# pypr/pysph

Hardware: AMD Instinct MI355X
Metric: particle-updates/sec (nnps.update + AccelerationEval.compute), WCSPH 3D, fp64 (higher is better)
Workload: dtype f64

## Files before the change

pysph_amd/csrc/sph_eval.hip:

```cpp
#include "sph_internal.h"
#include "sph_kernels.h"
#include "sph_pair.h"

#include <cfloat>
#include <cmath>
#include <type_traits>

struct EosArgs {
    int kind;
    double par[SPH_MAX_PAR];
    double *rho, *p, *cs;
    size_t start, stop;
    double *q[SPH_PROP_COUNT];
    uint32_t *tflag;
};

__device__ inline void jacobi_eigen3(double A[3][3], double V[3][3], double d[3])
{
    for (int i = 0; i < 3; i++) for (int j = 0; j < 3; j++) V[i][j] = (i == j) ? 1.0 : 0.0;
    for (int sweep = 0; sweep < 12; sweep++) {
        double off = fabs(A[0][1]) + fabs(A[0][2]) + fabs(A[1][2]);
        double diag = fabs(A[0][0]) + fabs(A[1][1]) + fabs(A[2][2]);
        if (off <= 1e-300 || off <= 1e-18 * diag) break;
#pragma unroll
// ... 334 lines not shown
    }
    const double rho = v[6];
    const double q = rho != 0.0 ? v[7] * (1.0 / (rho * rho)) : 0.0;
    const double srho = ((a.cls >> sl) & 1u) ? -rho : rho;
    if (!(rho > 0.0) && fabs(v[0]) < SPH_PARKED_MIN) atomicOr(a.rho_flag, 1u);
    double hp = 0.0;
    if (VH) hp = kernarg_read<const double *>(__builtin_offsetof(PackMArgs, prop) + ((size_t)8 * SPH_MAX_ARRAYS + sl) * sizeof(double *))[o];
    a.fpos[i] = make_float4((float)(v[0] - a.gmin[0]), (float)(v[1] - a.gmin[1]), (float)(v[2] - a.gmin[2]),
                            VH ? (float)(a.hr * hp) : (float)a.hr);
    double2 pc[PACK_MAXP];
#pragma unroll
    for (int k = 0; k < PACK_MAXP; k++) pc[k] = make_double2(0.0, 0.0);
    int np;
    if (VH && F32) {
        pc[0] = __builtin_bit_cast(double2, make_float4((float)(v[0] - a.gmin[0]), (float)(v[1] - a.gmin[1]), (float)(v[2] - a.gmin[2]), (float)hp));
        pc[1] = __builtin_bit_cast(double2, make_float4((float)v[3], (float)v[4], (float)v[5], (float)srho));
        np = 2;
    } else if (VH) {
        pc[0] = make_double2(v[0], v[1]); pc[1] = make_double2(v[2], hp);
        pc[2] = make_double2(v[3], v[4]); pc[3] = make_double2(v[5], srho);
        np = 4;
    } else if (F32) {
        pc[0] = __builtin_bit_cast(double2, make_float4((float)(v[0] - a.gmin[0]), (float)(v[1] - a.gmin[1]), (float)(v[2] - a.gmin[2]), (float)v[3]));
        pc[1] = __builtin_bit_cast(double2, make_float4((float)v[4], (float)v[5], (float)srho, (float)q));
        np = 2;
    } else {
        pc[0] = make_double2(v[0], v[1]); pc[1] = make_double2(v[2], v[3]);
        pc[2] = make_double2(v[4], v[5]); pc[3] = make_double2(srho, q);
        np = 4;
    }
    emit_pieces(a, i, pc, np);
}

template <class T> struct FamWCSPH_T {
    typedef T Real;
    static constexpr uint32_t CF0 = F_CONT | F_MOM | F_XSPH;
#ifndef SPH_WCSPH_MINB
#define SPH_WCSPH_MINB 4
#endif
    static constexpr int MINB = SPH_WCSPH_MINB;
    static constexpr int NA = 8;
    static constexpr int NR = 12;
    struct Params {
        T c0, alpha, beta, gx, gy, gz, eps;
        double *arho, *au, *av, *aw, *ax, *ay, *az, *dt_cfl, *dt_force;
    };
    struct Dest {
        T u, v, w, rho, p, cs, tmpi;
        T arho, au, av, aw, ax, ay, az, dt_cfl;
    };
    template <class A> static __device__ __forceinline__ void load(Dest &D, const T *a, const A &, uint32_t)
    {
        D.u = a[0]; D.v = a[1]; D.w = a[2]; D.rho = a[4]; D.tmpi = a[5]; D.cs = a[6]; D.p = a[7];
        D.arho = D.au = D.av = D.aw = D.ax = D.ay = D.az = T(0.0);
        D.dt_cfl = T(-1.0);
    }
    static constexpr bool PRED = true;
    template <int KK, bool UH, class A>
    static __device__ __forceinline__ void pair(Dest &D, const real4<T> &pi, const real4<T> &pj, T r2,
                                                const T (&s)[NA], uint32_t fl, const A &a, bool pass = true)
    {
        PairGeomT<T> g;
        constexpr bool MRG = SPH_MERGED_RSQ && sizeof(T) == 8 && KK != 4;
        T tt_m = T(0.0);
        if constexpr (MRG) {
            if (fl & F_MOM) tt_m = pair_geom_mom<KK, UH>(g, pi, pj, r2, T(0.5) * (D.rho + s[4]), a);
            else pair_geom<KK, UH>(g, pi, pj, r2, a);
        } else {
            pair_geom<KK, UH>(g, pi, pj, r2, a);
        }
        const T tg = pair_gradfac<KK, UH>(g);
        const T vij0 = D.u - s[0], vij1 = D.v - s[1], vij2 = D.w - s[2];
        const T vdotx = vij0 * g.xij[0] + vij1 * g.xij[1] + vij2 * g.xij[2];
        const T mj = pass ? s[3] : T(0.0);
        if (fl & F_CONT) D.arho = fma(mj * tg, vdotx, D.arho);
        if (fl & (F_MOM | F_XSPH)) {
            const T rhoij = T(0.5) * (D.rho + s[4]);
            T rhoij1;
            T wij = T(0.0);
            if (fl & (F_XSPH | F_TENSILE)) wij = pair_w<KK, UH>(g);
            if (fl & F_MOM) {
                const T re = r2 + g.eps;
                const T tt = MRG ? tt_m : fast_rcp(re * rhoij);
                const T inv_re = rhoij * tt;
                rhoij1 = re * tt;
                const T hv = g.hij * vdotx;
                const T muij = raw_min(hv, T(0.0)) * inv_re;
                const T cij = T(0.5) * (D.cs + s[6]);
                const T piij = (a.p.beta * muij - a.p.alpha * cij) * muij * rhoij1;
                const T dtv = fabs(hv * (g.rinv * g.rinv));
                D.dt_cfl = raw_max(D.dt_cfl, (r2 > T(1e-12) && pass) ? dtv : T(-1.0));
                const T tmpj = s[5];
                T tmp = D.tmpi + tmpj;
                if (fl & F_TENSILE) {
                    const T qd = (a.k.deltap * g.hij) * g.h1;
                    const T wdp = SphKernel<KK>::w(qd) * g.fac;
                    T fij = wij * fast_rcp(wdp);
                    fij = fij * fij;
                    fij = fij * fij;
                    const T Ri = D.p > 0 ? T(0.01) * D.tmpi : T(0.2) * fabs(D.tmpi);
                    const T Rj = s[7] > 0 ? T(0.01) * tmpj : T(0.2) * fabs(tmpj);
                    tmp = (D.tmpi + tmpj) + (Ri + Rj) * fij;
                }
                const T ft = -mj * (tmp + piij) * tg;
                D.au = fma(ft, g.xij[0], D.au);
                D.av = fma(ft, g.xij[1], D.av);
                D.aw = fma(ft, g.xij[2], D.aw);
            } else {
                rhoij1 = fast_rcp(rhoij);
            }
            if (fl & F_XSPH) {
                const T tmp = -a.p.eps * mj * wij * rhoij1;
                D.ax = fma(tmp, vij0, D.ax);
                D.ay = fma(tmp, vij1, D.ay);
                D.az = fma(tmp, vij2, D.az);
            }
        }
    }
    template <class A> static __device__ __forceinline__ void finish(Dest &D, const A &a, uint32_t o)
    {
        if (a.dflags & F_CONT) a.p.arho[o] = D.arho;
        if (a.dflags & F_MOM) {
            T au = D.au + a.p.gx, av = D.av + a.p.gy, aw = D.aw + a.p.gz;
            a.p.au[o] = au; a.p.av[o] = av; a.p.aw[o] = aw;
            a.p.dt_cfl[o] = D.dt_cfl < T(0.0) ? T(0.0) : D.dt_cfl + a.p.c0;
            a.p.dt_force[o] = au * au + av * av + aw * aw;
        }
        if (a.dflags & F_XSPH) {
            a.p.ax[o] = D.ax + D.u; a.p.ay[o] = D.ay + D.v; a.p.az[o] = D.az + D.w;
        }
    }
};
typedef FamWCSPH_T<double> FamWCSPH;

template <class T, bool UM = false> struct FamWCSPHE_T : FamWCSPH_T<T> {
    static constexpr bool EOSF = true;
    static constexpr bool UMASS = UM;
    static constexpr int NR = 8;
    struct Raw {
        typename std::conditional<sizeof(T) == 8, double2, float4>::type q[sizeof(T) == 8 ? 4 : 2];
    };
    template <class A> static __device__ __forceinline__ void load_raw(const A &a, uint32_t jg, Raw &r)
    {
        if constexpr (sizeof(T) == 8) {
            const double2 *p = reinterpret_cast<const double2 *>(a.rec) + (unsigned long long)jg * 4;
            r.q[0] = p[0]; r.q[1] = p[1]; r.q[2] = p[2]; r.q[3] = p[3];
        } else {
            const float4 *p = reinterpret_cast<const float4 *>(a.rec) + (unsigned long long)jg * 2;
            r.q[0] = p[0]; r.q[1] = p[1];
        }
    }
    template <class A> static __device__ __forceinline__ void decode(const A &a, const Raw &r, uint32_t fl, T mu, real4<T> &pj, T (&s)[8],
                                                                     int gk = 3)
    {
        T rho;
        if constexpr (sizeof(T) == 8) {
            pj.x = r.q[0].x; pj.y = r.q[0].y; pj.z = r.q[1].x; pj.w = 0.0;
            s[0] = r.q[1].y; s[1] = r.q[2].x; s[2] = r.q[2].y; s[3] = r.q[3].y; rho = r.q[3].x;
        } else {
            pj.x = r.q[0].x; pj.y = r.q[0].y; pj.z = r.q[0].z; pj.w = 0.f;
            s[0] = r.q[0].w; s[1] = r.q[1].x; s[2] = r.q[1].y; s[3] = r.q[1].w; rho = r.q[1].z;
        }
        s[4] = rho;
        s[5] = s[6] = s[7] = T(0.0);
        if constexpr (UM) {
            const T q = s[3];
            s[3] = mu;
            if (fl & F_MOM) {
                const T ratio = rho * (T)a.e_rho01;
                s[5] = q;
                s[6] = (T)a.e_c0 * tait_cs_power(ratio, gk);
            }
        } else
        if (fl & F_MOM) {
            const T ratio = rho * (T)a.e_rho01;
            T r7, r3;
            tait_powers(ratio, gk, r7, r3);
            const T p = (T)a.e_p0 + (T)a.e_B * (r7 - T(1.0));
            s[5] = rho != T(0.0) ? p * fast_rcp(rho * rho) : T(0.0);
            s[6] = (T)a.e_c0 * r3;
            s[7] = p;
        }
    }
    template <class A> static __device__ __forceinline__ void load_fused(const A &a, uint32_t jg, uint32_t fl, T mu, real4<T> &pj, T (&s)[8])
    {
        Raw r;
        load_raw(a, jg, r);
        decode(a, r, fl, mu, pj, s);
    }
};

template <class T, bool UM = false> struct FamWCSPHEG_T : FamWCSPHE_T<T, UM> {
    typedef FamWCSPHE_T<T, UM> Base;
    template <class A> static __device__ __forceinline__ void load_fused(const A &a, uint32_t jg, uint32_t fl, T mu, real4<T> &pj, T (&s)[8])
    {
        typename Base::Raw r;
        Base::load_raw(a, jg, r);
        Base::decode(a, r, fl, mu, pj, s, a.e_gk);
    }
};

template <class T> struct FamWCSPHV_T : FamWCSPH_T<T> {
    static constexpr bool EOSF = true;
    static constexpr int NR = 8;
    template <class A> static __device__ __forceinline__ void load_fused(const A &a, uint32_t jg, uint32_t fl, T mu, real4<T> &pj, T (&s)[8])
    {
        T rho;
        if constexpr (sizeof(T) == 8) {
            const double2 *p = reinterpret_cast<const double2 *>(a.rec) + (unsigned long long)jg * 4;
            const double2 q0 = p[0], q1 = p[1], q2 = p[2], q3 = p[3];
            pj.x = q0.x; pj.y = q0.y; pj.z = q1.x; pj.w = q1.y;
            s[0] = q2.x; s[1] = q2.y; s[2] = q3.x; rho = q3.y;
        } else {
            const float4 *p = reinterpret_cast<const float4 *>(a.rec) + (unsigned long long)jg * 2;
            const float4 q0 = p[0], q1 = p[1];
            pj.x = q0.x; pj.y = q0.y; pj.z = q0.z; pj.w = q0.w;
            s[0] = q1.x; s[1] = q1.y; s[2] = q1.z; rho = q1.w;
        }
        s[3] = mu;
        s[4] = rho;
// ... 550 lines not shown
    uint32_t o = a.d_perm[i];
    if (o < a.d_start || o >= a.d_stop) return;
    double4 pi = a.posh[a.d_off + i];
    typename Fam::Dest D;
    Fam::load(D, a.aux + (size_t)(a.d_off + i) * Fam::NA, a, o);
    uint32_t key = a.d_keys[i];
    int cx = key % a.nc[0];
    int t = key / a.nc[0];
    int cy = t % a.nc[1], cz = t / a.nc[1];
    double hi2 = a.radius_scale * pi.w;
    hi2 *= hi2;
    for (int s = 0; s < a.nsrc; s++) {
        const SrcDesc sd = a.src[s];
        for (int oz = -1; oz <= 1; oz++)
            for (int oy = -1; oy <= 1; oy++) {
                int yy = cy + oy, zz = cz + oz;
                if (yy < 0 || yy >= a.nc[1] || zz < 0 || zz >= a.nc[2]) continue;
                int xa = max(cx - 1, 0), xb = min(cx + 1, a.nc[0] - 1);
                uint32_t row = (uint32_t)(a.nc[0] * (yy + a.nc[1] * zz));
                uint32_t j0 = sd.cell_start[row + xa], j1 = sd.cell_start[row + xb + 1];
                for (uint32_t j = j0; j < j1; j++) {
                    double4 pj = a.posh[sd.off + j];
                    double hj2 = a.radius_scale * pj.w;
                    hj2 *= hj2;
                    double r2 = r2_exact(pi.x - pj.x, pi.y - pj.y, pi.z - pj.z);
                    if ((r2 < hi2) || (r2 < hj2)) {
                        double sj[Fam::NA];
                        load_aux<Fam>(sj, a.aux + (size_t)(sd.off + j) * Fam::NA);
                        Fam::template pair<KK, UH>(D, pi, pj, r2, sj, sd.flags, a);
                    }
                }
            }
    }
    Fam::finish(D, a, o);
}

static bool is_nosrc_kind(int k)
{
    return k == SPH_EQ_TAIT_EOS || k == SPH_EQ_TAIT_EOS_HG || k == SPH_EQ_TVF_STATE_EQUATION ||
           k == SPH_EQ_ISOTHERMAL_EOS || k == SPH_EQ_SOLID_ISOTHERMAL_EOS || k == SPH_EQ_MONAGHAN_ART_STRESS ||
           k == SPH_EQ_HOOKES_DEVIATORIC_STRESS_RATE;
}

static int need_prop(sph_ctx *c, int id, int prop, const char *who)
{
    if (!c->arr[id].prop[prop]) {
        sph_set_error("%s: array %d has no device copy of a required property (id %d); push it first", who, id, prop);
        return SPH_ERR_MISSING_PROP;
    }
    return SPH_OK;
}

static int run_nosrc(sph_ctx *c, const sph_equation &e, size_t start, size_t stop)
{
    if (stop <= start) return SPH_OK;
    DevArray &A = c->arr[e.dest];
    EosArgs a;
    a.kind = e.kind;
    memcpy(a.par, e.par, sizeof a.par);
    SPH_TRY(need_prop(c, e.dest, SPH_RHO, "EOS"));
    SPH_TRY(sph_array_ensure_prop(c, e.dest, SPH_P));
    a.rho = A.prop[SPH_RHO];
    a.p = A.prop[SPH_P];
    a.cs = nullptr;
    if (e.kind == SPH_EQ_TAIT_EOS || e.kind == SPH_EQ_TAIT_EOS_HG) {
        SPH_TRY(sph_array_ensure_prop(c, e.dest, SPH_CS));
        a.cs = A.prop[SPH_CS];
// ... 267 lines not shown
        case 3: LAUNCH(3); break;
        case 4: LAUNCH(4); break;
        }
#undef LAUNCH
        return SPH_OK;
    }
}

template <class Fam, bool UHV = true> static int launch_pair_fused(sph_ctx *c, int kk, const PairArgs<Fam> &a)
{
    if (a.nd == 0) return SPH_OK;
    constexpr bool FP32 = sizeof(typename Fam::Real) == 4;
    dim3 g2(div_up(4 * div_up(a.nd, 256), WPB)), b2(64 * WPB);
    uint32_t cf = a.src[0].flags;
    for (int j = 1; j < a.nsrc; j++) if (a.src[j].flags != cf) cf = 0;
    if (c->const_flags == 0) cf = 0;
    if constexpr (fam_rowlds<Fam>::value && UHV) {
        if (c->row_lds && !a.nl_mode && !a.face_mode) {
            dim3 g1(4 * div_up(a.nd, 256)), b1(64);
#define LAUNCHL(K)                                                                                              \
            if (cf == Fam::CF0) hipLaunchKernelGGL((k_pair_rowlds<Fam, K, Fam::CF0>), g1, b1, 0, c->stream, a); \
            else hipLaunchKernelGGL((k_pair_rowlds<Fam, K, 0>), g1, b1, 0, c->stream, a)
            switch (kk) {
            case 1: LAUNCHL(1); break;
            case 2: LAUNCHL(2); break;
            case 3: LAUNCHL(3); break;
            case 4: LAUNCHL(4); break;
            }
#undef LAUNCHL
            c->timers[T_N_ROWLDS].count++;
            return SPH_OK;
        }
    }
#define LAUNCHE(K)                                                                                                              \
    if (cf == Fam::CF0) hipLaunchKernelGGL((k_pair_wave<Fam, K, UHV, FP32, Fam::CF0>), g2, b2, (size_t)c->lds_pad, c->stream, a); \
    else hipLaunchKernelGGL((k_pair_wave<Fam, K, UHV, FP32, 0>), g2, b2, (size_t)c->lds_pad, c->stream, a)
    switch (kk) {
    case 1: LAUNCHE(1); break;
    case 2: LAUNCHE(2); break;
    case 3: LAUNCHE(3); break;
    case 4: LAUNCHE(4); break;
    }
#undef LAUNCHE
    return SPH_OK;
}

template <class Fam>
static void fill_common(sph_ctx *c, PairArgs<Fam> &a, const sph_kernel *K, double t)
{
    a.posh = c->posh.as<double4>();
    a.aux = c->aux.as<double>();
    a.rec = c->posh.as<double>();
    a.nrec = c->cur_nrec;
    a.fpos = c->fposb.as<float4>();
    a.dom_extent = fmax(fmax(c->xmax[0] - c->xmin[0], c->xmax[1] - c->xmin[1]), c->xmax[2] - c->xmin[2]);
    for (int k = 0; k < 3; k++) { a.nc[k] = c->nc[k]; a.xmin[k] = c->xmin[k]; }
    a.cell_size = c->cell_size;
    a.radius_scale = c->radius_scale;
    a.k.sigma = K->fac;
    a.k.deltap = K->deltap;
    a.k.dim = K->dim;
    a.t = t;
    a.dt = c->cur_dt;
    a.ablate = (int)c->ablate;
    a.dbg = c->count_iters ? c->dbgc.as<unsigned long long>() : nullptr;
    a.hu = 0.5 * (c->h_uniform + c->h_uniform);
    a.h1u = 1.0 / a.hu;
    a.facu = K->fac * a.h1u;
// ... 485 lines not shown
                const DevArray &S = c->arr[srcs[j]];
                a.src[a.nsrc++] = {S.cell_start.as<uint32_t>(), (uint32_t)off_of[j], sflags[j], S.fine_start.as<uint32_t>(), S.m_value, 0u};
            }
            for (int j = 0; j < nsrcs && phase != 1; j++) {
                const DevArray &S = c->arr[srcs[j]];
                if (S.g_n == 0) continue;
                a.src[a.nsrc++] = {S.g_cell_start.as<uint32_t>(), (uint32_t)(off_of[j] + S.n_binned), sflags[j],
                                   S.g_fine_start.as<uint32_t>(), S.m_value, 1u};
            }
            a.face_mode = c->split_pair ? phase : 0;
            a.d_off = (uint32_t)d_off; a.nd = (uint32_t)D.n_binned;
            a.d_mu = D.m_value;
            a.d_keys = D.keys_sorted.as<uint32_t>(); a.d_fkeys = D.fkeys_sorted.as<uint32_t>(); a.d_perm = D.perm.as<uint32_t>();
            set_tile_order(c, a, D);
            a.d_start = (uint32_t)start; a.d_stop = (uint32_t)stop; a.dflags = dflags;
            a.nl = nullptr; a.nl_mode = nl_mode;
            if (nl_mode) a.nl = c->nlbuf.as<uint32_t>();
            if (start == 0 && stop == D.n_real && D.n_binned == D.n && !any_ghosts) use_dest_list(c, a, D);
            if (eosf || eosv) {
                a.e_rho01 = 1.0 / g->eos_par[0]; a.e_c0 = g->eos_par[1];
                a.e_B = g->eos_par[0] * g->eos_par[1] * g->eos_par[1] / g->eos_par[2];
        a.e_gk = tait_gk(g->eos_par[2]);
                a.e_p0 = g->eos_par[3];
            }
            if (tvff) { a.e_p0 = g->eos_par[0]; a.e_rho01 = 1.0 / g->eos_par[1]; a.e_B = g->eos_par[2]; }
        };
        auto run_wcsph = [&](auto tag) -> int {
            typedef decltype(tag) F;
            PairArgs<F> a;
            memset(&a, 0, sizeof a);
            common(a);
            const sph_equation *me = eq_of[SPH_EQ_MOMENTUM], *xe = eq_of[SPH_EQ_XSPH];
            if (me) { a.p.c0 = me->par[0]; a.p.alpha = me->par[1]; a.p.beta = me->par[2]; a.p.gx = me->par[3]; a.p.gy = me->par[4]; a.p.gz = me->par[5]; }
            if (xe) a.p.eps = xe->par[0];
            if (dflags & F_CONT) { SPH_TRY(ensure_out(c, dst, {SPH_ARHO})); a.p.arho = D.prop[SPH_ARHO]; }
            if (dflags & F_MOM) {
                SPH_TRY(ensure_out(c, dst, {SPH_AU, SPH_AV, SPH_AW, SPH_DT_CFL, SPH_DT_FORCE}));
                a.p.au = D.prop[SPH_AU]; a.p.av = D.prop[SPH_AV]; a.p.aw = D.prop[SPH_AW];
                a.p.dt_cfl = D.prop[SPH_DT_CFL]; a.p.dt_force = D.prop[SPH_DT_FORCE];
            }
            if (dflags & F_XSPH) {
                SPH_TRY(ensure_out(c, dst, {SPH_AX, SPH_AY, SPH_AZ}));
                a.p.ax = D.prop[SPH_AX]; a.p.ay = D.prop[SPH_AY]; a.p.az = D.prop[SPH_AZ];
            }
            if constexpr (std::is_same<F, FamWCSPHV_T<typename F::Real>>::value) return launch_pair_fused<F, false>(c, K->kind, a);
            else if constexpr (fam_eosf<F>::value) return launch_pair_fused<F>(c, K->kind, a);
            else return launch_pair<F>(c, K->kind, a);
        };
        auto run_density = [&](auto tag) -> int {
            typedef decltype(tag) F;
            PairArgs<F> a;
            memset(&a, 0, sizeof a);
            common(a);
            SPH_TRY(ensure_out(c, dst, {SPH_RHO}));
            a.p.rho = D.prop[SPH_RHO];
            if (dflags & F_TVFSD) { SPH_TRY(ensure_out(c, dst, {SPH_VOL})); a.p.V = D.prop[SPH_VOL]; }
            if ((dflags & F_SD) && (dflags & F_TVFSD)) { sph_set_error("both SummationDensity flavours on one destination"); return SPH_ERR_UNSUPPORTED; }
            return launch_pair<F>(c, K->kind, a);
        };
        auto run_vgrad = [&](auto tag) -> int {
            typedef decltype(tag) F;
            PairArgs<F> a;
            memset(&a, 0, sizeof a);
            common(a);
            static const int vp[9] = {SPH_V00, SPH_V01, SPH_V02, SPH_V10, SPH_V11, SPH_V12, SPH_V20, SPH_V21, SPH_V22};
            if ((dflags & F_VG2) && (dflags & F_VG3)) { sph_set_error("both VelocityGradient2D and 3D on one destination"); return SPH_ERR_UNSUPPORTED; }
// ... 356 lines not shown
```

pysph_amd/csrc/sph_kernels.h:

```cpp
#pragma once

#include <hip/hip_runtime.h>

template <int KIND> struct SphKernel;

__device__ __forceinline__ double raw_max(double a, double b)
{
    double r;
    asm("v_max_f64 %0, %1, %2" : "=v"(r) : "v"(a), "v"(b));
    return r;
}
__device__ __forceinline__ double raw_min(double a, double b)
{
    double r;
    asm("v_min_f64 %0, %1, %2" : "=v"(r) : "v"(a), "v"(b));
    return r;
}
__device__ __forceinline__ float raw_max(float a, float b) { return fmaxf(a, b); }
__device__ __forceinline__ float raw_min(float a, float b) { return fminf(a, b); }


template <class R> __device__ __forceinline__ R kernel_norm(R sigma, R h1, int dim)
{
    R f = sigma * h1;
    if (dim > 1) f *= h1;
    if (dim > 2) f *= h1;
    return f;
}

template <> struct SphKernel<1> {
    static constexpr bool HAS_DWQ = false;
    template <bool INSUP = false, class R> static __device__ __forceinline__ R dwq(R) { return R(0); }
    template <bool INSUP = false, class R> static __device__ __forceinline__ R w(R q)
    {
        R t2 = R(2) - q;
        R a = R(0.25) * t2 * t2 * t2;
        R b = R(1) - R(1.5) * q * q * (R(1) - R(0.5) * q);
        return (!INSUP && q > R(2)) ? R(0) : (q > R(1) ? a : b);
    }
    template <bool INSUP = false, class R> static __device__ __forceinline__ R dw(R q)
    {
        R t2 = R(2) - q;
        R a = R(-0.75) * t2 * t2;
        R b = R(-3) * q * (R(1) - R(0.75) * q);
        return (!INSUP && q > R(2)) ? R(0) : (q > R(1) ? a : b);
    }
};

template <> struct SphKernel<2> {
    static constexpr bool HAS_DWQ = true;
    template <bool INSUP = false, class R> static __device__ __forceinline__ R dwq(R q)
    {
// ... 48 lines not shown
```

pysph_amd/csrc/sph_pair.h:

```cpp
#pragma once

#include <hip/hip_runtime.h>
#include <cstdint>

#include "sphhip.h"
#include "sph_kernels.h"

template <class T> __device__ __forceinline__ T r2_exact(T dx, T dy, T dz)
{
#pragma clang fp contract(off)
    const T a = dx * dx, b = dy * dy, c = dz * dz;
    return (a + b) + c;
}

template <class T> struct Real4Of;
template <> struct Real4Of<double> { typedef double4 type; };
template <> struct Real4Of<float> { typedef float4 type; };
template <class T> using real4 = typename Real4Of<T>::type;


struct KernelConst {
    double sigma;
    double deltap;
    int dim;
// ... 33 lines not shown
    SrcDesc src[SPH_MAX_ARRAYS];
    const double4 *posh;
    const double *aux;
    const double *rec;
    int nrec;
    const float4 *fpos;
    double dom_extent;
    uint32_t d_off, nd;
    double d_mu;
    const uint32_t *d_keys, *d_fkeys, *d_perm;
    const uint8_t *d_slot;
    const uint32_t *d_tile_order;
    const uint32_t *d_list;
    int face_mode, gfx_lo, gfx_hi;
    int row_mod3;
    uint32_t d_start, d_stop;
    int nc[3];
    double xmin[3];
    double cell_size;
    double radius_scale;
    KernelConst k;
    uint32_t dflags;
    unsigned long long *dbg;
    int ablate;
    int skip_init;
    int skip_post;
    double t, dt;
    double hu, h1u, facu, epsu, hr2u;
    uint32_t *nl;
    int nl_mode;
    int norm_masks;
    double e_rho01, e_c0, e_B, e_p0;
    int e_gk;
    typename Fam::Params p;
};

template <class F, class = void> struct fam_merged { static constexpr bool value = false; };
template <class F> struct fam_merged<F, decltype((void)F::MERGED)> { static constexpr bool value = F::MERGED; };

template <class V> __device__ __forceinline__ V kernarg_read(size_t byte_offset)
{
    typedef const char __attribute__((address_space(4))) *kptr;
    const kptr ka = (kptr)__builtin_amdgcn_kernarg_segment_ptr();
    return *reinterpret_cast<const V __attribute__((address_space(4))) *>(ka + byte_offset);
}

template <class F, class = void> struct fam_token { static constexpr bool value = false; };
template <class F> struct fam_token<F, decltype((void)F::TOKEN)> { static constexpr bool value = F::TOKEN; };

template <class F, class = void> struct fam_eosf { static constexpr bool value = false; };
template <class F> struct fam_eosf<F, decltype((void)F::EOSF)> { static constexpr bool value = F::EOSF; };


#ifndef SPH_NEWTON_STEPS
#define SPH_NEWTON_STEPS 1
#endif
__device__ __forceinline__ double fast_rcp(double d)
{
    double x = __builtin_amdgcn_rcp(d);
    double e = fma(-d, x, 1.0);
    x = fma(x, e, x);
    if (SPH_NEWTON_STEPS > 1) {
        e = fma(-d, x, 1.0);
        x = fma(x, e, x);
    }
    return x;
}
__device__ __forceinline__ void fast_sqrt_rsqrt(double a, double &s, double &rs)
{
    a = raw_max(a, 1e-300);
    double y = __builtin_amdgcn_rsq(a);
    double g = a * y, h = 0.5 * y;
    double r = fma(-h, g, 0.5);
    g = fma(g, r, g);
    h = fma(h, r, h);
    if (SPH_NEWTON_STEPS > 1) {
        r = fma(-h, g, 0.5);
        g = fma(g, r, g);
        h = fma(h, r, h);
    }
    s = g;
    rs = h + h;
}
__device__ __forceinline__ float fast_rcp(float d) { return __builtin_amdgcn_rcpf(d); }
__device__ __forceinline__ void fast_sqrt_rsqrt(float a, float &s, float &rs)
{
    a = fmaxf(a, 1e-35f);
    rs = __builtin_amdgcn_rsqf(a);
    s = a * rs;
}

template <class T> struct PairGeomT {
    T xij[3];
    T r2, rij, rinv, hij, h1, q, fac, eps;
};
typedef PairGeomT<double> PairGeom;

template <int KK, bool UH, class T, class A>
__device__ __forceinline__ void pair_geom(PairGeomT<T> &g, const real4<T> &pi, const real4<T> &pj, T r2, const A &a)
{
    g.xij[0] = pi.x - pj.x; g.xij[1] = pi.y - pj.y; g.xij[2] = pi.z - pj.z;
    g.r2 = r2;
    constexpr bool EXACT_Q = (KK == 4);
    if (EXACT_Q) {
        g.rij = sqrt(r2);
        g.rinv = g.rij > T(0) ? T(1) / g.rij : T(0);
    } else {
        fast_sqrt_rsqrt(r2, g.rij, g.rinv);
    }
    if (UH) {
        g.hij = (T)a.hu; g.h1 = (T)a.h1u; g.fac = (T)a.facu; g.eps = (T)a.epsu;
    } else {
        g.hij = T(0.5) * (pi.w + pj.w);
        g.h1 = EXACT_Q ? T(1) / g.hij : fast_rcp(g.hij);
        g.fac = kernel_norm((T)a.k.sigma, g.h1, a.k.dim);
        g.eps = T(0.01) * g.hij * g.hij;
    }
    g.q = g.rij * g.h1;
}
#ifndef SPH_MERGED_RSQ
#define SPH_MERGED_RSQ 0
#endif
template <int KK, bool UH, class A>
__device__ __forceinline__ double pair_geom_mom(PairGeomT<double> &g, const double4 &pi, const double4 &pj, double r2, double rhoij, const A &a)
{
    typedef double T;
    g.xij[0] = pi.x - pj.x; g.xij[1] = pi.y - pj.y; g.xij[2] = pi.z - pj.z;
    g.r2 = r2;
    if (UH) {
        g.hij = (T)a.hu; g.h1 = (T)a.h1u; g.fac = (T)a.facu; g.eps = (T)a.epsu;
    } else {
        g.hij = T(0.5) * (pi.w + pj.w);
        g.h1 = fast_rcp(g.hij);
        g.fac = kernel_norm((T)a.k.sigma, g.h1, a.k.dim);
        g.eps = T(0.01) * g.hij * g.hij;
    }
    const T P = (r2 + g.eps) * rhoij;
    const T r2c = raw_max(r2, 1e-300);
    const T aa = r2c * (P * P);
    const T y = __builtin_amdgcn_rsq(aa);
    T gg = aa * y, hh = 0.5 * y;
    const T rr = fma(-hh, gg, 0.5);
    hh = fma(hh, rr, hh);
    const T t = hh + hh;
    g.rinv = t * P;
    g.rij = r2c * g.rinv;
    g.q = g.rij * g.h1;
    return t * g.rij;
}

template <int KK, bool UH, class T> __device__ __forceinline__ T pair_w(const PairGeomT<T> &g) { return SphKernel<KK>::template w<UH>(g.q) * g.fac; }
template <int KK, bool UH, class T> __device__ __forceinline__ T pair_gradh(const PairGeomT<T> &g, int dim)
{
    return -g.fac * g.h1 * (SphKernel<KK>::template dw<UH>(g.q) * g.q + SphKernel<KK>::template w<UH>(g.q) * (T)dim);
}
template <int KK, bool UH, class T> __device__ __forceinline__ T pair_gradfac(const PairGeomT<T> &g)
{
    T t;
    if (SphKernel<KK>::HAS_DWQ) t = SphKernel<KK>::template dwq<UH>(g.q) * (g.fac * g.h1 * g.h1);
    else t = SphKernel<KK>::template dw<UH>(g.q) * (g.fac * g.h1) * g.rinv;
    return g.rij > T(1e-12) ? t : T(0);
}

template <class Fam, bool UH>
__device__ __forceinline__ void load_record(const double *__restrict__ rj, uint32_t fl, double4 &pj, double (&s)[Fam::NA])
{
    pj = *reinterpret_cast<const double4 *>(rj);
#pragma unroll
    for (int k = 0; k < Fam::NA; k++) s[k] = rj[4 + k];
}

template <class Fam, class T>
__device__ __forceinline__ void load_record_f32(const float *__restrict__ rj, real4<T> &pj, T (&s)[Fam::NA])
{
    constexpr int NF = (4 + Fam::NA + 3) & ~3;
    float f[NF];
    const float4 *r4 = reinterpret_cast<const float4 *>(rj);
#pragma unroll
    for (int q = 0; q < NF / 4; q++) { const float4 t = r4[q]; f[4 * q] = t.x; f[4 * q + 1] = t.y; f[4 * q + 2] = t.z; f[4 * q + 3] = t.w; }
    pj.x = f[0]; pj.y = f[1]; pj.z = f[2]; pj.w = f[3];
#pragma unroll
    for (int k = 0; k < Fam::NA; k++) s[k] = f[4 + k];
}

template <int NA, class T>
__device__ __forceinline__ void pin_record(const real4<T> &pj, const T (&s)[NA])
{
    asm volatile("" ::"v"(pj.x), "v"(pj.y), "v"(pj.z));
#pragma unroll
    for (int k = 0; k < NA; k++)
        if (!__builtin_constant_p(s[k])) asm volatile("" ::"v"(s[k]));
}

__device__ __forceinline__ uint32_t xcd_tile(uint32_t b, uint32_t nb)
// ... 10 lines not shown
    return __builtin_amdgcn_readfirstlane(v);
}

#ifdef SPH_PROFILING
#define ABLATE(a) ((a).ablate)
#define DBGC(a) ((a).dbg)
#else
#define ABLATE(a) 0
#define DBGC(a) ((unsigned long long *)nullptr)
#endif

#define AMAXLEN 96

typedef float f2 __attribute__((ext_vector_type(2)));

#ifndef SPH_WLQ
#define SPH_WLQ 10
#endif
#ifndef SPH_WCAP_UH
#define SPH_WCAP_UH 184
#endif
#define WLQ SPH_WLQ
#define WCAP_UH SPH_WCAP_UH
#define WCAP_VH 136
#define WCSL 96
#define NLW (64 * (1 + 3 * WLQ))
#define NL_NONE 0xFFFFFFFFu
#define XWIN (SPH_NSUB + 1)

#ifndef WPB
#define WPB 1
#endif

template <class Fam, int KK, bool UH, bool F32 = false, uint32_t CF = 0>
__global__ __launch_bounds__(64 * WPB, Fam::MINB) void k_pair_wave(PairArgs<Fam> a)
{
    typedef typename Fam::Real T;
    static_assert(F32 || sizeof(T) == 8, "fp32 arithmetic reads fp32 records");
    const uint32_t NR = (uint32_t)a.nrec;
    constexpr int WCAP = UH ? WCAP_UH : WCAP_VH;
    constexpr int TS = WCAP + 8;
    __shared__ __attribute__((aligned(16))) float tile_[WPB][(UH ? 3 : 4) * TS];
    __shared__ unsigned short csl_[WPB][WCSL];
    __shared__ unsigned long long smask_[WPB][WLQ][64];
    __shared__ uint32_t sjb_[WPB][WLQ][64];
    const int wv = __builtin_amdgcn_readfirstlane((int)(threadIdx.x >> 6));
    float *const tile = tile_[wv];
    float *const tx = tile, *const ty = tile + TS, *const tz = tile + 2 * TS, *const tw = tile + (UH ? 0 : 3 * TS);
    unsigned short *const csl = csl_[wv];
    unsigned long long (*const smask)[64] = smask_[wv];
    uint32_t (*const sjb)[64] = sjb_[wv];

    const int t = threadIdx.x & 63;
    const uint32_t wt = xcd_tile(blockIdx.x, gridDim.x) * WPB + (uint32_t)wv;
    uint32_t dtile = wt >> 2;
    if (dtile * 256u >= a.nd) return;
    if (a.d_tile_order) dtile = a.d_tile_order[dtile];
    const uint32_t tbase = dtile * 256u + (wt & 3u) * 64u;
    const uint32_t i = tbase + t;
    if (tbase >= a.nd) return;
    const bool valid = i < a.nd;
    uint32_t ic = valid ? i : a.nd - 1;
    if (a.d_list) ic = a.d_list[ic];
    const uint32_t o = a.d_perm[ic];
    uint32_t slot = 0;
    bool active;
    if constexpr (fam_merged<Fam>::value) {
        slot = a.d_slot[ic];
        const unsigned long long rg = kernarg_read<unsigned long long>(__builtin_offsetof(PairArgs<Fam>, p) + Fam::rng_offset(slot));
        active = valid && o >= (uint32_t)rg && o < (uint32_t)(rg >> 32);
    } else {
        active = valid && o >= a.d_start && o < a.d_stop;
    }
    const uint32_t fkey = a.d_fkeys[ic];
    const uint32_t key = fkey / SPH_NSUB;
    const int ncx = a.nc[0], ncy = a.nc[1], ncz = a.nc[2];
    const int row = key / ncx;
    const int cx = (int)(key % ncx) * SPH_NSUB + (int)(fkey % SPH_NSUB);
    bool facew = true;
    if (a.face_mode != 0 || a.gfx_lo > -0x7fffffff || a.gfx_hi < 0x7fffffff) {
        int mn = active ? cx : 0x7fffffff, mx = active ? cx : -0x7fffffff;
#pragma unroll
        for (int o = 32; o > 0; o >>= 1) { mn = min(mn, __shfl_xor(mn, o, 64)); mx = max(mx, __shfl_xor(mx, o, 64)); }
        mn = __builtin_amdgcn_readfirstlane(mn); mx = __builtin_amdgcn_readfirstlane(mx);
        facew = mn <= mx && (mn - XWIN <= a.gfx_lo || mx + XWIN >= a.gfx_hi);
        if (mn > mx && !a.nl_mode) return;
        if (a.face_mode == 1 && facew) return;
        if (a.face_mode == 2 && !facew) return;
    }
    real4<T> pi;
    typename Fam::Dest D;
    uint32_t wtok = 0;
    if constexpr (fam_token<Fam>::value) wtok = Fam::wave_token(a);
    T cur_mu = (T)a.d_mu;
    auto fetch = [&](uint32_t jg, uint32_t flags, real4<T> &pj, T (&sj)[Fam::NA]) {
        if constexpr (fam_token<Fam>::value) Fam::load_fused(a, jg, flags, cur_mu, pj, sj, wtok);
        else if constexpr (fam_eosf<Fam>::value) Fam::load_fused(a, jg, flags, cur_mu, pj, sj);
        else if constexpr (F32) load_record_f32<Fam, T>(reinterpret_cast<const float *>(a.rec) + (unsigned long long)jg * NR, pj, sj);
        else load_record<Fam, UH>(a.rec + (unsigned long long)jg * NR, flags, pj, sj);
    };
    {
        T sd_[Fam::NA];
        fetch(a.d_off + ic, a.dflags, pi, sd_);
        if (UH) pi.w = (T)a.hu;
        if constexpr (fam_merged<Fam>::value) Fam::load(D, sd_, a, o, slot);
        else Fam::load(D, sd_, a, o);
    }
    const int nfx = ncx * SPH_NSUB;
    const T hi_r = (T)a.radius_scale * pi.w;
    const T hi2 = UH ? (T)a.hr2u : hi_r * hi_r;
    const int row_first = __builtin_amdgcn_readfirstlane(row), row_last = __builtin_amdgcn_readlane(row, 63);
    if (DBGC(a) && t == 0) atomicAdd(DBGC(a) + 2, 1ull);

    auto do_pair = [&](uint32_t jg, uint32_t flags) {
        real4<T> pj;
        T sj[Fam::NA];
        fetch(jg, flags, pj, sj);
        pin_record<Fam::NA, T>(pj, sj);
        T hj2 = hi2;
        if (!UH) { hj2 = (T)a.radius_scale * pj.w; hj2 *= hj2; }
        const T r2 = r2_exact<T>(pi.x - pj.x, pi.y - pj.y, pi.z - pj.z);
        if (((r2 < hi2) || (r2 < hj2)) && ABLATE(a) != 1) Fam::template pair<KK, UH>(D, pi, pj, r2, sj, flags, a);
    };

    int cq = 0;
    auto phase2 = [&](uint32_t flags) {
        unsigned long long m = 0;
        uint32_t jb = 0;
        int q = 0;
        if (cq > 0 && ABLATE(a) != 2) { m = smask[0][t]; jb = sjb[0][t]; }
        const uint32_t self = a.d_off + ic;
        if (__any(m != 0)) {
            if (DBGC(a) && t == 0) atomicAdd(DBGC(a) + 1, 1ull);
            do {
                if (DBGC(a) && t == 0) atomicAdd(DBGC(a), 1ull);
                const bool has = m != 0;
                uint32_t j = has ? jb + (uint32_t)__builtin_ctzll(m) : self;
                m &= m - 1;
                if (m == 0 && q + 1 < cq) { ++q; m = smask[q][t]; jb = sjb[q][t]; }
                if (ABLATE(a) == 3) j = self;
                if constexpr (Fam::PRED) {
                    real4<T> pj;
                    T sj[Fam::NA];
                    fetch(j, flags, pj, sj);
                    T hj2 = hi2;
                    if (!UH) { hj2 = (T)a.radius_scale * pj.w; hj2 *= hj2; }
                    const T r2 = r2_exact<T>(pi.x - pj.x, pi.y - pj.y, pi.z - pj.z);
                    const bool pass = has && ((r2 < hi2) || (r2 < hj2)) && ABLATE(a) != 1;
                    Fam::template pair<KK, UH>(D, pi, pj, r2, sj, flags, a, pass);
                } else {
                    if (has) do_pair(j, flags);
                }
            } while (__any(m != 0));
        }
        cq = 0;
    };

    uint32_t *const nlw = a.nl_mode ? a.nl + (size_t)wt * NLW : nullptr;
    bool reuse = false, unsaved = false;
    if (a.nl_mode == 2) {
        const uint32_t nq = nlw[t];
        reuse = !__any(nq == NL_NONE);
        if (reuse) {
            const uint32_t off0 = a.src[0].off;
            const int nqmax = wave_max_i32((int)nq);
            for (int q = 0; q < nqmax; q++) {
                const uint32_t *w = nlw + 64 * (1 + 3 * q) + t;
                smask[q][t] = (unsigned long long)w[0] | ((unsigned long long)w[64] << 32);
                sjb[q][t] = w[128] + off0;
            }
            __builtin_amdgcn_fence(__ATOMIC_ACQ_REL, "wavefront");
            cq = active ? (int)nq : 0;
        }
    }

    for (int s = 0; s < a.nsrc; s++) {
    const SrcDesc sd = a.src[s];
    if (sd.ghost && !facew) continue;
    const uint32_t fl = CF ? CF : sd.flags;
    cur_mu = (T)sd.mu;
    int R = row_first, st = 0, part_resume = 0;
    uint32_t tb_resume = 0;
    bool resumed = false;
    for (;;) {
    bool more = false;
    for (; R <= row_last && !more && !reuse && ABLATE(a) != 6; R++, st = 0) {
// ... 110 lines not shown
                    if (__any(cq + (m0 != 0) + (m2 != 0) > WLQ)) { more = true; break; }
                    if (m0) { smask[cq][t] = m0; sjb[cq][t] = jb0; cq++; }
                    if (m2) { smask[cq][t] = m2; sjb[cq][t] = jb0 + 64u; cq++; }
                }
                __builtin_amdgcn_fence(__ATOMIC_ACQ_REL, "wavefront");
                if (more) { tb_resume = tb; part_resume = part; break; }
            }
            if (more) break;
        }
        if (more) break;
    }
    if (a.nl_mode == 1 && s == 0) {
        if (unsaved || more) nlw[t] = NL_NONE;
        else {
            __builtin_amdgcn_fence(__ATOMIC_ACQ_REL, "wavefront");
            nlw[t] = (uint32_t)cq;
            const int nqmax = wave_max_i32(cq);
            for (int q = 0; q < nqmax; q++) {
                uint32_t *w = nlw + 64 * (1 + 3 * q) + t;
                const unsigned long long m = q < cq ? smask[q][t] : 0ull;
                w[0] = (uint32_t)m; w[64] = (uint32_t)(m >> 32);
                w[128] = q < cq ? sjb[q][t] - sd.off : 0u;
            }
        }
    }
    phase2(fl);
    if (!more) break;
    unsaved = true;
    resumed = true;
    }
    }
    if (active) {
        if constexpr (fam_merged<Fam>::value) Fam::finish(D, a, o, slot);
        else Fam::finish(D, a, o);
    }
}


template <class F, class = void> struct fam_rowlds { static constexpr bool value = false; };
template <class F> struct fam_rowlds<F, decltype((void)F::ROWLDS)> { static constexpr bool value = F::ROWLDS; };

#ifndef SPH_WCAP_L
#define SPH_WCAP_L 96
#endif
#define WCAP_L SPH_WCAP_L

template <class Fam, int KK, uint32_t CF = 0>
__global__ __launch_bounds__(64, Fam::MINB) void k_pair_rowlds(PairArgs<Fam> a)
{
    typedef typename Fam::Real T;
    typedef typename Fam::Piece Piece;
    constexpr int NP = Fam::PIECES;
    constexpr int TS = WCAP_L + 8;
    static_assert(WCAP_L <= AMAXLEN && WCAP_L % 8 == 0, "one part per tile");
    __shared__ __attribute__((aligned(16))) float tile[3 * TS];
    __shared__ unsigned short csl[WCSL];
    __shared__ __attribute__((aligned(16))) Piece recs[WCAP_L * NP];
    float *const tx = tile, *const ty = tile + TS, *const tz = tile + 2 * TS;

    const int t = threadIdx.x & 63;
    const uint32_t wt = xcd_tile(blockIdx.x, gridDim.x);
    uint32_t dtile = wt >> 2;
    if (dtile * 256u >= a.nd) return;
    if (a.d_tile_order) dtile = a.d_tile_order[dtile];
    const uint32_t tbase = dtile * 256u + (wt & 3u) * 64u;
    const uint32_t i = tbase + t;
// ... 146 lines not shown
```

Before: 2.001 billion.

## Trim WCSPH pair arithmetic, use 32-bit record offsets, split neighbor masks into words

Several micro-optimizations go into the fp64 WCSPH pair kernel. The artificial viscosity term becomes a single fma, using beta and a precomputed -alpha/2 held in registers. The dt_cfl max uses v_max_f64 with an abs modifier and NaN masking, and accumulates a quarter-scaled value that is multiplied by 4 at finish. Pass-gating moves from the mass to the gradient factor and the XSPH weight. It also adds a kernel variant that computes record addresses with 32-bit offsets when the buffer is under 4 GiB, and rewrites the phase-2 neighbor mask walk to use 32-bit words with ctz instead of 64-bit ctzll. Together these aim to cut VALU instruction count and 64-bit address arithmetic per neighbor pair, at the cost of more template variants and subtle changes in NaN and rounding behaviour.

```diff
diff --git a/pysph_amd/csrc/sph_eval.hip b/pysph_amd/csrc/sph_eval.hip
--- a/pysph_amd/csrc/sph_eval.hip
+++ b/pysph_amd/csrc/sph_eval.hip
@@ -390,6 +390,9 @@
     emit_pieces(a, i, pc, np);
 }
 
+template <class P, class = void> struct has_nhalpha { static constexpr bool value = false; };
+template <class P> struct has_nhalpha<P, decltype((void)P::nhalpha)> { static constexpr bool value = true; };
+
 template <class T> struct FamWCSPH_T {
     typedef T Real;
     static constexpr uint32_t CF0 = F_CONT | F_MOM | F_XSPH;
@@ -402,18 +405,27 @@
     struct Params {
         T c0, alpha, beta, gx, gy, gz, eps;
         double *arho, *au, *av, *aw, *ax, *ay, *az, *dt_cfl, *dt_force;
+        T nhalpha;
     };
     struct Dest {
         T u, v, w, rho, p, cs, tmpi;
         T arho, au, av, aw, ax, ay, az, dt_cfl;
+        T kbeta, knha;
     };
-    template <class A> static __device__ __forceinline__ void load(Dest &D, const T *a, const A &, uint32_t)
-    {
+    template <class A> static __device__ __forceinline__ void load(Dest &D, const T *a, const A &args, uint32_t)
+    {
+        if constexpr (has_nhalpha<typename A::ParamsT>::value && GATE1) {
+            D.kbeta = args.p.beta; D.knha = args.p.nhalpha;
+            asm volatile("" : "+v"(D.kbeta), "+v"(D.knha));
+        }
         D.u = a[0]; D.v = a[1]; D.w = a[2]; D.rho = a[4]; D.tmpi = a[5]; D.cs = a[6]; D.p = a[7];
         D.arho = D.au = D.av = D.aw = D.ax = D.ay = D.az = T(0.0);
         D.dt_cfl = T(-1.0);
     }
     static constexpr bool PRED = true;
+    static constexpr bool GATE1 = sizeof(T) == 8;
+    static constexpr bool FINISH_KK = true;
+    template <int KK> static constexpr bool dt_quarter() { return sizeof(T) == 8 && KK != 4 && !SPH_MERGED_RSQ; }
     template <int KK, bool UH, class A>
     static __device__ __forceinline__ void pair(Dest &D, const real4<T> &pi, const real4<T> &pj, T r2,
                                                 const T (&s)[NA], uint32_t fl, const A &a, bool pass = true)
@@ -427,10 +439,10 @@
         } else {
             pair_geom<KK, UH>(g, pi, pj, r2, a);
         }
-        const T tg = pair_gradfac<KK, UH>(g);
+        const T tg = pair_gradfac<KK, UH>(g, GATE1 ? pass : true);
         const T vij0 = D.u - s[0], vij1 = D.v - s[1], vij2 = D.w - s[2];
         const T vdotx = vij0 * g.xij[0] + vij1 * g.xij[1] + vij2 * g.xij[2];
-        const T mj = pass ? s[3] : T(0.0);
+        const T mj = (GATE1 || pass) ? s[3] : T(0.0);
         if (fl & F_CONT) D.arho = fma(mj * tg, vdotx, D.arho);
         if (fl & (F_MOM | F_XSPH)) {
             const T rhoij = T(0.5) * (D.rho + s[4]);
@@ -444,10 +456,16 @@
                 rhoij1 = re * tt;
                 const T hv = g.hij * vdotx;
                 const T muij = raw_min(hv, T(0.0)) * inv_re;
-                const T cij = T(0.5) * (D.cs + s[6]);
-                const T piij = (a.p.beta * muij - a.p.alpha * cij) * muij * rhoij1;
-                const T dtv = fabs(hv * (g.rinv * g.rinv));
-                D.dt_cfl = raw_max(D.dt_cfl, (r2 > T(1e-12) && pass) ? dtv : T(-1.0));
+                T piij;
+                if constexpr (GATE1) piij = fma(D.kbeta, muij, D.knha * (D.cs + s[6])) * muij * rhoij1;
+                else piij = (a.p.beta * muij - a.p.alpha * (T(0.5) * (D.cs + s[6]))) * muij * rhoij1;
+                if constexpr (GATE1) {
+                    const T dtv = dt_quarter<KK>() ? hv * (g.rinvh * g.rinvh) : hv * (g.rinv * g.rinv);
+                    D.dt_cfl = raw_max_abs(D.dt_cfl, nan_unless(r2 > T(1e-12) && pass, dtv));
+                } else {
+                    const T dtv = fabs(hv * (g.rinv * g.rinv));
+                    D.dt_cfl = raw_max(D.dt_cfl, (r2 > T(1e-12) && pass) ? dtv : T(-1.0));
+                }
                 const T tmpj = s[5];
                 T tmp = D.tmpi + tmpj;
                 if (fl & F_TENSILE) {
@@ -468,20 +486,22 @@
                 rhoij1 = fast_rcp(rhoij);
             }
             if (fl & F_XSPH) {
-                const T tmp = -a.p.eps * mj * wij * rhoij1;
+                const T wx = (!GATE1 || pass) ? wij : T(0.0);
+                const T tmp = -a.p.eps * mj * wx * rhoij1;
                 D.ax = fma(tmp, vij0, D.ax);
                 D.ay = fma(tmp, vij1, D.ay);
                 D.az = fma(tmp, vij2, D.az);
             }
         }
     }
-    template <class A> static __device__ __forceinline__ void finish(Dest &D, const A &a, uint32_t o)
+    template <int KK = 4, class A> static __device__ __forceinline__ void finish(Dest &D, const A &a, uint32_t o)
     {
         if (a.dflags & F_CONT) a.p.arho[o] = D.arho;
         if (a.dflags & F_MOM) {
             T au = D.au + a.p.gx, av = D.av + a.p.gy, aw = D.aw + a.p.gz;
             a.p.au[o] = au; a.p.av[o] = av; a.p.aw[o] = aw;
-            a.p.dt_cfl[o] = D.dt_cfl < T(0.0) ? T(0.0) : D.dt_cfl + a.p.c0;
+            const T dtm = dt_quarter<KK>() ? T(4.0) * D.dt_cfl : D.dt_cfl;
+            a.p.dt_cfl[o] = D.dt_cfl < T(0.0) ? T(0.0) : dtm + a.p.c0;
             a.p.dt_force[o] = au * au + av * av + aw * aw;
         }
         if (a.dflags & F_XSPH) {
@@ -498,15 +518,15 @@
     struct Raw {
         typename std::conditional<sizeof(T) == 8, double2, float4>::type q[sizeof(T) == 8 ? 4 : 2];
     };
-    template <class A> static __device__ __forceinline__ void load_raw(const A &a, uint32_t jg, Raw &r)
-    {
-        if constexpr (sizeof(T) == 8) {
-            const double2 *p = reinterpret_cast<const double2 *>(a.rec) + (unsigned long long)jg * 4;
-            r.q[0] = p[0]; r.q[1] = p[1]; r.q[2] = p[2]; r.q[3] = p[3];
-        } else {
-            const float4 *p = reinterpret_cast<const float4 *>(a.rec) + (unsigned long long)jg * 2;
-            r.q[0] = p[0]; r.q[1] = p[1];
-        }
+    template <bool O32 = false, class A> static __device__ __forceinline__ void load_raw(const A &a, uint32_t jg, Raw &r)
+    {
+        typedef typename std::remove_reference<decltype(r.q[0])>::type Q;
+        constexpr uint32_t RB = sizeof(Raw);
+        const Q *p;
+        if constexpr (O32) p = reinterpret_cast<const Q *>(reinterpret_cast<const char *>(a.rec) + (uint32_t)(jg * RB));
+        else p = reinterpret_cast<const Q *>(a.rec) + (unsigned long long)jg * (RB / 16);
+        r.q[0] = p[0]; r.q[1] = p[1];
+        if constexpr (sizeof(T) == 8) { r.q[2] = p[2]; r.q[3] = p[3]; }
     }
     template <class A> static __device__ __forceinline__ void decode(const A &a, const Raw &r, uint32_t fl, T mu, real4<T> &pj, T (&s)[8],
                                                                      int gk = 3)
@@ -540,10 +560,10 @@
             s[7] = p;
         }
     }
-    template <class A> static __device__ __forceinline__ void load_fused(const A &a, uint32_t jg, uint32_t fl, T mu, real4<T> &pj, T (&s)[8])
+    template <bool O32 = false, class A> static __device__ __forceinline__ void load_fused(const A &a, uint32_t jg, uint32_t fl, T mu, real4<T> &pj, T (&s)[8])
     {
         Raw r;
-        load_raw(a, jg, r);
+        load_raw<O32>(a, jg, r);
         decode(a, r, fl, mu, pj, s);
     }
 };
@@ -1160,7 +1180,8 @@
                 }
             }
     }
-    Fam::finish(D, a, o);
+    if constexpr (fam_finish_kk<Fam>::value) Fam::template finish<KK>(D, a, o);
+    else Fam::finish(D, a, o);
 }
 
 static bool is_nosrc_kind(int k)
@@ -1494,8 +1515,11 @@
             return SPH_OK;
         }
     }
+    constexpr bool CAN32 = std::is_same<Fam, FamWCSPHE_T<typename Fam::Real, true>>::value && UHV;
+    const bool o32 = CAN32 && c->posh.bytes < (1ull << 32);
 #define LAUNCHE(K)                                                                                                              \
-    if (cf == Fam::CF0) hipLaunchKernelGGL((k_pair_wave<Fam, K, UHV, FP32, Fam::CF0>), g2, b2, (size_t)c->lds_pad, c->stream, a); \
+    if (cf == Fam::CF0 && o32) hipLaunchKernelGGL((k_pair_wave<Fam, K, UHV, FP32, Fam::CF0, CAN32>), g2, b2, (size_t)c->lds_pad, c->stream, a); \
+    else if (cf == Fam::CF0) hipLaunchKernelGGL((k_pair_wave<Fam, K, UHV, FP32, Fam::CF0>), g2, b2, (size_t)c->lds_pad, c->stream, a); \
     else hipLaunchKernelGGL((k_pair_wave<Fam, K, UHV, FP32, 0>), g2, b2, (size_t)c->lds_pad, c->stream, a)
     switch (kk) {
     case 1: LAUNCHE(1); break;
@@ -2047,6 +2071,7 @@
             common(a);
             const sph_equation *me = eq_of[SPH_EQ_MOMENTUM], *xe = eq_of[SPH_EQ_XSPH];
             if (me) { a.p.c0 = me->par[0]; a.p.alpha = me->par[1]; a.p.beta = me->par[2]; a.p.gx = me->par[3]; a.p.gy = me->par[4]; a.p.gz = me->par[5]; }
+            if (me) a.p.nhalpha = (typename F::Real)(-0.5 * me->par[1]);
             if (xe) a.p.eps = xe->par[0];
             if (dflags & F_CONT) { SPH_TRY(ensure_out(c, dst, {SPH_ARHO})); a.p.arho = D.prop[SPH_ARHO]; }
             if (dflags & F_MOM) {
diff --git a/pysph_amd/csrc/sph_kernels.h b/pysph_amd/csrc/sph_kernels.h
--- a/pysph_amd/csrc/sph_kernels.h
+++ b/pysph_amd/csrc/sph_kernels.h
@@ -18,6 +18,18 @@
 }
 __device__ __forceinline__ float raw_max(float a, float b) { return fmaxf(a, b); }
 __device__ __forceinline__ float raw_min(float a, float b) { return fminf(a, b); }
+__device__ __forceinline__ double raw_max_abs(double a, double b)
+{
+    double r;
+    asm("v_max_f64 %0, %1, |%2|" : "=v"(r) : "v"(a), "v"(b));
+    return r;
+}
+__device__ __forceinline__ float raw_max_abs(float a, float b) { return fmaxf(a, fabsf(b)); }
+__device__ __forceinline__ double nan_unless(bool keep, double x)
+{
+    return __hiloint2double(keep ? __double2hiint(x) : 0x7ff80000, __double2loint(x));
+}
+__device__ __forceinline__ float nan_unless(bool keep, float x) { return keep ? x : __builtin_nanf(""); }
 
 
 template <class R> __device__ __forceinline__ R kernel_norm(R sigma, R h1, int dim)
diff --git a/pysph_amd/csrc/sph_pair.h b/pysph_amd/csrc/sph_pair.h
--- a/pysph_amd/csrc/sph_pair.h
+++ b/pysph_amd/csrc/sph_pair.h
@@ -89,6 +89,7 @@
     int norm_masks;
     double e_rho01, e_c0, e_B, e_p0;
     int e_gk;
+    typedef typename Fam::Params ParamsT;
     typename Fam::Params p;
 };
 
@@ -104,6 +105,9 @@
 
 template <class F, class = void> struct fam_token { static constexpr bool value = false; };
 template <class F> struct fam_token<F, decltype((void)F::TOKEN)> { static constexpr bool value = F::TOKEN; };
+
+template <class F, class = void> struct fam_finish_kk { static constexpr bool value = false; };
+template <class F> struct fam_finish_kk<F, decltype((void)F::FINISH_KK)> { static constexpr bool value = F::FINISH_KK; };
 
 template <class F, class = void> struct fam_eosf { static constexpr bool value = false; };
 template <class F> struct fam_eosf<F, decltype((void)F::EOSF)> { static constexpr bool value = F::EOSF; };
@@ -123,7 +127,7 @@
     }
     return x;
 }
-__device__ __forceinline__ void fast_sqrt_rsqrt(double a, double &s, double &rs)
+__device__ __forceinline__ void fast_sqrt_rsqrt(double a, double &s, double &rs, double &rsh)
 {
     a = raw_max(a, 1e-300);
     double y = __builtin_amdgcn_rsq(a);
@@ -138,18 +142,21 @@
     }
     s = g;
     rs = h + h;
+    rsh = h;
 }
 __device__ __forceinline__ float fast_rcp(float d) { return __builtin_amdgcn_rcpf(d); }
-__device__ __forceinline__ void fast_sqrt_rsqrt(float a, float &s, float &rs)
+__device__ __forceinline__ void fast_sqrt_rsqrt(float a, float &s, float &rs, float &rsh)
 {
     a = fmaxf(a, 1e-35f);
     rs = __builtin_amdgcn_rsqf(a);
     s = a * rs;
+    rsh = 0.5f * rs;
 }
 
 template <class T> struct PairGeomT {
     T xij[3];
     T r2, rij, rinv, hij, h1, q, fac, eps;
+    T rinvh;
 };
 typedef PairGeomT<double> PairGeom;
 
@@ -162,8 +169,9 @@
     if (EXACT_Q) {
         g.rij = sqrt(r2);
         g.rinv = g.rij > T(0) ? T(1) / g.rij : T(0);
+        g.rinvh = T(0.5) * g.rinv;
     } else {
-        fast_sqrt_rsqrt(r2, g.rij, g.rinv);
+        fast_sqrt_rsqrt(r2, g.rij, g.rinv, g.rinvh);
     }
     if (UH) {
         g.hij = (T)a.hu; g.h1 = (T)a.h1u; g.fac = (T)a.facu; g.eps = (T)a.epsu;
@@ -201,6 +209,7 @@
     hh = fma(hh, rr, hh);
     const T t = hh + hh;
     g.rinv = t * P;
+    g.rinvh = T(0.5) * g.rinv;
     g.rij = r2c * g.rinv;
     g.q = g.rij * g.h1;
     return t * g.rij;
@@ -211,12 +220,12 @@
 {
     return -g.fac * g.h1 * (SphKernel<KK>::template dw<UH>(g.q) * g.q + SphKernel<KK>::template w<UH>(g.q) * (T)dim);
 }
-template <int KK, bool UH, class T> __device__ __forceinline__ T pair_gradfac(const PairGeomT<T> &g)
+template <int KK, bool UH, class T> __device__ __forceinline__ T pair_gradfac(const PairGeomT<T> &g, bool gate = true)
 {
     T t;
     if (SphKernel<KK>::HAS_DWQ) t = SphKernel<KK>::template dwq<UH>(g.q) * (g.fac * g.h1 * g.h1);
     else t = SphKernel<KK>::template dw<UH>(g.q) * (g.fac * g.h1) * g.rinv;
-    return g.rij > T(1e-12) ? t : T(0);
+    return (g.rij > T(1e-12) && gate) ? t : T(0);
 }
 
 template <class Fam, bool UH>
@@ -293,11 +302,12 @@
 #define WPB 1
 #endif
 
-template <class Fam, int KK, bool UH, bool F32 = false, uint32_t CF = 0>
+template <class Fam, int KK, bool UH, bool F32 = false, uint32_t CF = 0, bool O32 = false>
 __global__ __launch_bounds__(64 * WPB, Fam::MINB) void k_pair_wave(PairArgs<Fam> a)
 {
     typedef typename Fam::Real T;
     static_assert(F32 || sizeof(T) == 8, "fp32 arithmetic reads fp32 records");
+    static_assert(!O32 || (fam_eosf<Fam>::value && !fam_token<Fam>::value), "32-bit record offsets: families with load_fused<O32>");
     const uint32_t NR = (uint32_t)a.nrec;
     constexpr int WCAP = UH ? WCAP_UH : WCAP_VH;
     constexpr int TS = WCAP + 8;
@@ -356,6 +366,7 @@
     T cur_mu = (T)a.d_mu;
     auto fetch = [&](uint32_t jg, uint32_t flags, real4<T> &pj, T (&sj)[Fam::NA]) {
         if constexpr (fam_token<Fam>::value) Fam::load_fused(a, jg, flags, cur_mu, pj, sj, wtok);
+        else if constexpr (fam_eosf<Fam>::value && O32) Fam::template load_fused<true>(a, jg, flags, cur_mu, pj, sj);
         else if constexpr (fam_eosf<Fam>::value) Fam::load_fused(a, jg, flags, cur_mu, pj, sj);
         else if constexpr (F32) load_record_f32<Fam, T>(reinterpret_cast<const float *>(a.rec) + (unsigned long long)jg * NR, pj, sj);
         else load_record<Fam, UH>(a.rec + (unsigned long long)jg * NR, flags, pj, sj);
@@ -386,19 +397,28 @@
 
     int cq = 0;
     auto phase2 = [&](uint32_t flags) {
-        unsigned long long m = 0;
-        uint32_t jb = 0;
-        int q = 0;
-        if (cq > 0 && ABLATE(a) != 2) { m = smask[0][t]; jb = sjb[0][t]; }
+        uint32_t mw = 0, mo = 0, jb = 0;
+        const unsigned long long *pm = &smask[0][t];
+        const uint32_t *pj = &sjb[0][t];
+        const unsigned long long *const pe = pm + 64 * (ABLATE(a) != 2 ? cq : 0);
+        auto step = [&]() {
+            if (mo == 0 && pm < pe) {
+                const unsigned long long m = *pm;
+                mw = (uint32_t)m; mo = (uint32_t)(m >> 32); jb = *pj;
+                pm += 64; pj += 64;
+            }
+            if (mw == 0) { mw = mo; mo = 0; jb += 32u; }
+        };
+        step();
         const uint32_t self = a.d_off + ic;
-        if (__any(m != 0)) {
+        if (__any(mw != 0)) {
             if (DBGC(a) && t == 0) atomicAdd(DBGC(a) + 1, 1ull);
             do {
                 if (DBGC(a) && t == 0) atomicAdd(DBGC(a), 1ull);
-                const bool has = m != 0;
-                uint32_t j = has ? jb + (uint32_t)__builtin_ctzll(m) : self;
-                m &= m - 1;
-                if (m == 0 && q + 1 < cq) { ++q; m = smask[q][t]; jb = sjb[q][t]; }
+                const bool has = mw != 0;
+                uint32_t j = has ? jb + (uint32_t)__builtin_ctz(mw) : self;
+                mw &= mw - 1;
+                if (mw == 0) step();
                 if (ABLATE(a) == 3) j = self;
                 if constexpr (Fam::PRED) {
                     real4<T> pj;
@@ -412,7 +432,7 @@
                 } else {
                     if (has) do_pair(j, flags);
                 }
-            } while (__any(m != 0));
+            } while (__any(mw != 0));
         }
         cq = 0;
     };
@@ -589,6 +609,7 @@
     }
     if (active) {
         if constexpr (fam_merged<Fam>::value) Fam::finish(D, a, o, slot);
+        else if constexpr (fam_finish_kk<Fam>::value) Fam::template finish<KK>(D, a, o);
         else Fam::finish(D, a, o);
     }
 }
```

After: 1.997 billion (median of 2 runs). About the same (-0.2%).
